# josiahls/pybullet-gym

Measured on AMD Instinct MI355X. Metric: env steps/sec (whole node) at N parallel envs, Ant + Humanoid, 1/2/4/8 MI355X, higher is better.
Workload: dtype f64

## Files before the change

### pybullet-gym_amd/csrc/pbg_robot.hip

```cpp
#include <hip/hip_runtime.h>

#include "pbg_launch.h"
#include "pbg_step.hip"
#include "pbg_team.hip"
#include "pbg_gang.hip"

#ifndef PBG_ROBOT
#error "compile with -DPBG_ROBOT=<robot struct name>"
#endif
#define PBG_CAT2(a, b) a##b
#define PBG_CAT(a, b) PBG_CAT2(a, b)
#define PBG_FN(prefix) PBG_CAT(prefix, PBG_ROBOT)

namespace pbg {
using R = pbg_models::PBG_ROBOT;
using R64 = F64<R>;
using R64L = F64L<R>;

static inline unsigned blocks(int n, int b) { return (unsigned)((n + b - 1) / b); }

static int kernel_attrs(const void* fn, Geometry* g) {
  hipFuncAttributes a{};
  const hipError_t e = hipFuncGetAttributes(&a, fn);
  g->vgprs = e == hipSuccess ? a.numRegs : -1;
  g->scratch_bytes = e == hipSuccess ? (int)a.localSizeBytes : -1;
  return (int)e;
}

template <class RR>
static int plan_team(int n_envs, int cus, Geometry* g) {
  if constexpr (Team<RR>::ok) {
    using RW = TRows<RR, 16>;
    constexpr int ES = 16;
    constexpr size_t WB = sizeof(real_t<RR>);
    const int wgs = (n_envs + ES - 1) / ES;
    const int wpc = (wgs + cus - 1) / cus;
    const size_t budget = (size_t)163840 / (size_t)(wpc > 0 ? wpc : 1);
    long words = (long)(budget / ((size_t)ES * WB)) - RW::HEAD;
    int cap = (int)(words / RW::W);
    if (cap > RW::MR) cap = RW::MR;
    if (cap < 0) cap = 0;
    size_t per_env = (size_t)RW::HEAD + (size_t)cap * RW::W;
    if (per_env < (size_t)(2 * RR::NL + 2 * RR::NJ)) per_env = 2 * RR::NL + 2 * RR::NJ;
    g->team = 4;
    g->env_words = 0;
    g->block = 64;
    g->lds_rows = cap;
    g->lds_bytes = (size_t)ES * WB * per_env;
    g->scratch_words_per_env = RW::WORDS;
    g->word_bytes = (int)WB;
    const void* fn = (const void*)team_step_kernel<RR, 16>;
    const int e = (int)hipFuncSetAttribute(fn, hipFuncAttributeMaxDynamicSharedMemorySize, (int)g->lds_bytes);
    return e ? e : kernel_attrs(fn, g);
  } else {
    (void)n_envs; (void)cus; (void)g;
    return (int)hipErrorInvalidValue;
  }
}
template <class RR>
static bool launch_team(const Buffers& B, const StepIO& io, float* scratch, const Geometry& g, hipStream_t s) {
  if constexpr (Team<RR>::ok) {
    if (g.team != 4) return false;
    hipLaunchKernelGGL((team_step_kernel<RR, 16>), dim3(blocks(4 * B.n, 64)), dim3(64), g.lds_bytes, s, B, io, scratch,
                       g.lds_rows);
    return true;
  } else {
    (void)B; (void)io; (void)scratch; (void)g; (void)s;
    return false;
  }
}

template <class RR, int T>
constexpr bool gang_ok() {
  constexpr bool f64 = sizeof(real_t<RR>) == 8;
  return (RR::kind == 0 || RR::kind >= 2) && (!RR::harder || FP<RR>::NF > 0) && (T == 16 || gang32_ok<RR>()) &&
         !(f64 && gang_big<RR>() && T != 16);
}
template <class RR, int T>
constexpr bool gang_repl() {
  return T == 16 && !RR::harder && (sizeof(real_t<RR>) == 4 || RR::NDOF < 8);
}
template <class RR, int T>
static int plan_gang_t(int n_envs, int cus, Geometry* g) {
  if constexpr (gang_ok<RR, T>()) {
    using G = Gang<RR, T>;
    constexpr long WB = (long)sizeof(real_t<RR>);
    constexpr int EPB = gang_block<RR, T>() / T;
    static_assert(4L * GangTabs<RR>::WORDS + WB * EPB * ((G::FIXED + G::MIN_CONTACT_WORDS + 3L) & ~3L) <= 163840L,
                  "gang env regions exceed the CU's LDS");
    auto region = [&](int c) {
      const int w = G::FIXED + (c * G::PERC > G::MIN_CONTACT_WORDS ? c * G::PERC : G::MIN_CONTACT_WORDS);
      return (w + G::REGION_ALIGN - 1) & ~(G::REGION_ALIGN - 1);
    };
    const int wgs = (n_envs + EPB - 1) / EPB;
    int wpc = (wgs + cus - 1) / cus;
    const long fit0 = 163840L / (4L * (long)GangTabs<RR>::WORDS + WB * EPB * (long)region(0));
    if (wpc > fit0) wpc = fit0 > 0 ? (int)fit0 : 1;
    long budget = 163840L / (long)(wpc > 0 ? wpc : 1) - 4L * (long)GangTabs<RR>::WORDS;
    if (budget < 0) budget = 0;
    long words = budget / (long)(EPB * WB) - G::FIXED;
    int cap = (int)(words / G::PERC);
    if (cap > G::MAXC) cap = G::MAXC;
    if (cap < 0) cap = 0;
    while (cap > 0 && (long)region(cap) * EPB * WB > budget) cap--;
    constexpr bool REPL = gang_repl<RR, T>();
    g->gang_dist = !REPL || RR::NDOF >= 8 || (size_t)n_envs * T > (size_t)64 * 4 * cus;
    if ((g->force_dist == 0 || g->force_dist == 1) && REPL) g->gang_dist = g->force_dist;
    g->team = T;
    g->block = gang_block<RR, T>();
    g->lds_rows = cap;
    g->env_words = region(cap);
    g->lds_bytes = 4 * (size_t)GangTabs<RR>::WORDS + (size_t)WB * (size_t)EPB * (size_t)g->env_words;
    if (g->lds_bytes > (size_t)163840) return (int)hipErrorInvalidConfiguration;
    g->scratch_words_per_env = G::GWORDS;
    g->word_bytes = (int)WB;
    const void* fn;
    if constexpr (REPL)
      fn = g->gang_dist ? (const void*)gang_step_kernel<RR, T, true> : (const void*)gang_step_kernel<RR, T, false>;
    else
      fn = (const void*)gang_step_kernel<RR, T, true>;
    const int e = (int)hipFuncSetAttribute(fn, hipFuncAttributeMaxDynamicSharedMemorySize, (int)g->lds_bytes);
    return e ? e : kernel_attrs(fn, g);
  } else {
    (void)n_envs; (void)cus; (void)g;
    return (int)hipErrorInvalidValue;
  }
}
template <class RR>
static int plan_gang(int n_envs, int cus, Geometry* g, int lanes) {
  if (lanes < 0) lanes = 16;
  if (lanes == 32) return plan_gang_t<RR, 32>(n_envs, cus, g);
  return plan_gang_t<RR, 16>(n_envs, cus, g);
}
template <class RR, int T>
static bool launch_gang_t(const Buffers& B, const StepIO& io, float* scratch, const Geometry& g, hipStream_t s) {
  if constexpr (gang_ok<RR, T>()) {
    const dim3 grid(blocks(B.n, gang_block<RR, T>() / T)), blk(gang_block<RR, T>());
    if constexpr (gang_repl<RR, T>()) {
      if (!g.gang_dist) {
        hipLaunchKernelGGL((gang_step_kernel<RR, T, false>), grid, blk, g.lds_bytes, s, B, io, scratch, g.lds_rows,
                           g.env_words);
        return true;
      }
    }
    hipLaunchKernelGGL((gang_step_kernel<RR, T, true>), grid, blk, g.lds_bytes, s, B, io, scratch, g.lds_rows, g.env_words);
    return true;
  } else {
    (void)B; (void)io; (void)scratch; (void)g; (void)s;
    return false;
  }
}
template <class RR>
static bool launch_gang(const Buffers& B, const StepIO& io, float* scratch, const Geometry& g, hipStream_t s) {
  if (g.team == 16) return launch_gang_t<RR, 16>(B, io, scratch, g, s);
  if (g.team == 32) return launch_gang_t<RR, 32>(B, io, scratch, g, s);
  return false;
}

template <class RR>
constexpr bool lane_ok() {
#ifdef PBG_DEV_GANG_ONLY
  return false;
#else
  return RR::NS <= 128;
#endif
}
template <class RR>
static int plan_lane(int n_envs, int cus, Geometry* g) {
  if constexpr (lane_ok<RR>()) {
    g->team = 1;
    g->env_words = 0;
    const int per_cu = (n_envs + cus - 1) / cus;
    int b = 16;
    while (b < per_cu && b < 64) b *= 2;
    const int wgs = (n_envs + b - 1) / b;
    const int wpc = (wgs + cus - 1) / cus;
    const size_t budget = (size_t)163840 / (size_t)(wpc > 0 ? wpc : 1);
    using RW = Rows<RR, 64>;
    constexpr size_t WB = sizeof(real_t<RR>);
    long words = (long)(budget / ((size_t)b * WB)) - RW::NC - RW::LIMW;
    int cap = (int)(words / RW::W);
    if (cap > RW::MR) cap = RW::MR;
    if (cap < 0) cap = 0;
    g->block = b;
    g->lds_rows = cap;
    g->lds_bytes = (size_t)b * WB * ((size_t)RW::LIMW + (size_t)cap * RW::W + RW::NC);
    g->scratch_words_per_env = RW::WORDS;
    g->word_bytes = (int)WB;
    const void* fn = b == 64 ? (const void*)step_kernel<RR, 64> : (b == 32 ? (const void*)step_kernel<RR, 32> : (const void*)step_kernel<RR, 16>);
    const int e = (int)hipFuncSetAttribute(fn, hipFuncAttributeMaxDynamicSharedMemorySize, (int)g->lds_bytes);
    return e ? e : kernel_attrs(fn, g);
  } else {
    (void)n_envs; (void)cus; (void)g;
    return (int)hipErrorInvalidValue;
  }
}
template <class RR>
static int launch_lane(const Buffers& B, const StepIO& io, float* scratch, const Geometry& g, hipStream_t s) {
  if constexpr (lane_ok<RR>()) {
    const dim3 grid(blocks(B.n, g.block)), blk(g.block);
    if (g.block == 64) hipLaunchKernelGGL((step_kernel<RR, 64>), grid, blk, g.lds_bytes, s, B, io, scratch, g.lds_rows);
    else if (g.block == 32) hipLaunchKernelGGL((step_kernel<RR, 32>), grid, blk, g.lds_bytes, s, B, io, scratch, g.lds_rows);
    else hipLaunchKernelGGL((step_kernel<RR, 16>), grid, blk, g.lds_bytes, s, B, io, scratch, g.lds_rows);
    return (int)hipGetLastError();
  } else {
    (void)B; (void)io; (void)scratch; (void)g; (void)s;
    return (int)hipErrorInvalidValue;
  }
}

template <class RR>
constexpr bool team64_ok() { return Team<RR>::ok; }
int PBG_FN(plan_team64_)(int n_envs, int cus, Geometry* g);
bool PBG_FN(launch_team64_)(const Buffers& B, const StepIO& io, float* scratch, const Geometry& g, hipStream_t s);
int PBG_FN(debug_stamps_t64_)(unsigned long long* host_out);
#ifdef PBG_TEAM64_TU
int PBG_FN(debug_stamps_t64_)(unsigned long long* host_out) {
#ifdef PBG_STAMPS
  if (hipMemcpyFromSymbol(host_out, HIP_SYMBOL(g_stamps), sizeof(unsigned long long) * 16) != hipSuccess) return -3;
  unsigned long long z[16] = {0};
  if (hipMemcpyToSymbol(HIP_SYMBOL(g_stamps), z, sizeof(z)) != hipSuccess) return -3;
  return 0;
#else
  (void)host_out;
  return -1;
#endif
}
#ifdef PBG_TRACE64
extern "C" int pbg_debug_trace64(double* host_out) {
  if (hipMemcpyFromSymbol(host_out, HIP_SYMBOL(g_trace64), sizeof(g_trace64)) != hipSuccess) return -3;
  return (int)(sizeof(g_trace64) / sizeof(double));
}
#endif
int PBG_FN(plan_team64_)(int n_envs, int cus, Geometry* g) {
  if constexpr (team64_ok<R64>()) return plan_team<R64>(n_envs, cus, g);
  else { (void)n_envs; (void)cus; (void)g; return (int)hipErrorInvalidValue; }
}
bool PBG_FN(launch_team64_)(const Buffers& B, const StepIO& io, float* scratch, const Geometry& g, hipStream_t s) {
  if constexpr (team64_ok<R64>()) return launch_team<R64>(B, io, scratch, g, s);
  else { (void)B; (void)io; (void)scratch; (void)g; (void)s; return false; }
}
#else

int PBG_FN(plan_)(int n_envs, int cus, int mode, Geometry* g) {
  if (Team<R>::ok && mode == 1) return plan_team<R>(n_envs, cus, g);
  if (R::kind != 1 && (mode >= 1 || !lane_ok<R>())) return plan_gang<R>(n_envs, cus, g, g->gang_lanes);
  return plan_lane<R>(n_envs, cus, g);
}

int PBG_FN(launch_step_)(const Buffers& B, const StepIO& io, float* scratch, const Geometry& g, hipStream_t s) {
  if (launch_team<R>(B, io, scratch, g, s)) return (int)hipGetLastError();
  if (launch_gang<R>(B, io, scratch, g, s)) return (int)hipGetLastError();
  return launch_lane<R>(B, io, scratch, g, s);
}

int PBG_FN(launch_reset_)(const Buffers& B, const ResetIO& io, hipStream_t s) {
  hipLaunchKernelGGL(reset_kernel<R>, dim3(blocks(B.n, 64)), dim3(64), 0, s, B, io);
  return (int)hipGetLastError();
}

int PBG_FN(launch_get_state_)(const Buffers& B, double* phys, double* aux, hipStream_t s) {
  hipLaunchKernelGGL(get_state_kernel<R>, dim3(blocks(B.n, 64)), dim3(64), 0, s, B, phys, aux);
  return (int)hipGetLastError();
}

int PBG_FN(launch_set_state_)(const Buffers& B, const double* phys, const double* aux, hipStream_t s) {
  hipLaunchKernelGGL(set_state_kernel<R>, dim3(blocks(B.n, 64)), dim3(64), 0, s, B, phys, aux);
  return (int)hipGetLastError();
}

int PBG_FN(launch_pack_)(int n, const double* in, double* out, hipStream_t s) {
  hipLaunchKernelGGL(pack_kernel<R>, dim3(blocks(n, 64)), dim3(64), 0, s, n, in, out);
  return (int)hipGetLastError();
}

int PBG_FN(plan64_)(int n_envs, int cus, int mode, Geometry* g) {
  if (team64_ok<R64>() && mode == 1) return PBG_FN(plan_team64_)(n_envs, cus, g);
  if constexpr (gang_ok<R64, 16>()) {
    if (mode != 0) {
      if (g->gang_lanes == 32 || (g->gang_lanes < 0 && gang_ok<R64, 32>())) {
        if constexpr (gang_ok<R64, 32>()) return plan_gang_t<R64, 32>(n_envs, cus, g);
        else return (int)hipErrorInvalidValue;
      }
      return plan_gang_t<R64, 16>(n_envs, cus, g);
    }
  }
  return plan_lane<R64L>(n_envs, cus, g);
}
int PBG_FN(launch_step64_)(const Buffers& B, const StepIO& io, float* scratch, const Geometry& g, hipStream_t s) {
  if (PBG_FN(launch_team64_)(B, io, scratch, g, s)) return (int)hipGetLastError();
  if (launch_gang<R64>(B, io, scratch, g, s)) return (int)hipGetLastError();
  return launch_lane<R64L>(B, io, scratch, g, s);
}
int PBG_FN(launch_reset64_)(const Buffers& B, const ResetIO& io, hipStream_t s) {
  hipLaunchKernelGGL(reset_kernel<R64>, dim3(blocks(B.n, 64)), dim3(64), 0, s, B, io);
  return (int)hipGetLastError();
}
int PBG_FN(launch_get_state64_)(const Buffers& B, double* phys, double* aux, hipStream_t s) {
  hipLaunchKernelGGL(get_state_kernel<R64>, dim3(blocks(B.n, 64)), dim3(64), 0, s, B, phys, aux);
  return (int)hipGetLastError();
}
int PBG_FN(launch_set_state64_)(const Buffers& B, const double* phys, const double* aux, hipStream_t s) {
  hipLaunchKernelGGL(set_state_kernel<R64>, dim3(blocks(B.n, 64)), dim3(64), 0, s, B, phys, aux);
  return (int)hipGetLastError();
}

int PBG_FN(debug_stamps_)(unsigned long long* host_out) {
#ifdef PBG_STAMPS
  if (hipMemcpyFromSymbol(host_out, HIP_SYMBOL(g_stamps), sizeof(unsigned long long) * 16) != hipSuccess) return -3;
  unsigned long long z[16] = {0};
  if (hipMemcpyToSymbol(HIP_SYMBOL(g_stamps), z, sizeof(z)) != hipSuccess) return -3;
  unsigned long long t64[16];
  if (PBG_FN(debug_stamps_t64_)(t64) == 0)
    for (int i = 0; i < 16; i++) host_out[i] += t64[i];
  return 0;
#else
  (void)host_out;
  return -1;
#endif
}
#endif
}
```

### pybullet-gym_amd/csrc/pbg_team.hip

```cpp

namespace pbg {

#define PBG_QUAD_SYNC                                    \
  {                                                      \
    __builtin_amdgcn_fence(__ATOMIC_RELEASE, "wavefront"); \
    __builtin_amdgcn_wave_barrier();                     \
    __builtin_amdgcn_fence(__ATOMIC_ACQUIRE, "wavefront"); \
  }

#ifdef PBG_TRACE64
#define PBG_TRACE_PH 8
__device__ double g_trace64[256][PBG_TRACE_PH][8];
#define TRACE64(ph, i, v) \
  do { if constexpr (sizeof(Sc) == 8) g_trace64[(blockIdx.x * 64 + threadIdx.x) & 255][ph][i] = (double)(v); } while (0)
#else
#define TRACE64(ph, i, v) do {} while (0)
#endif

template <int N, class S = float>
struct BTab {
  S v[N > 0 ? N : 1][4];
};
template <int N>
struct BTabI {
// ... 974 lines not shown
        fwd6(Lbb, Ldb, y6);
        Sc D2 = 0.f;
  #pragma unroll
        for (int gg = 0; gg < 6; gg++) { D2 += y6[gg] * y6[gg]; }
        Sc z[NDB];
  #pragma unroll
        for (int a = 0; a < NDB; a++) z[a] = 0.f;
        rw.put(3 * n0 + dir, -1, z, y6, D2 > Sc(1e-12) ? fast_rcp(D2) : 0.f,
               dir == 0 ? (pos_target(dist, P.k_contact, P.k_sep)) : 0.f, (Sc)R::slot_mu[sl]);
      }
      n0++;
    });
    detect_branch();
  } else {
    static_for<0, T::NS0>([&](auto sl_c) {
      constexpr int sl = decltype(sl_c)::value;
      if (!((base_bits >> sl) & 1u)) return;
      const f3 cc = O + mulc(Rb, (Sc)R::slot_point[sl][0], (Sc)R::slot_point[sl][1], (Sc)R::slot_point[sl][2]);
      const Sc rad = (Sc)R::slot_radius[sl];
      const Sc dist = cc.z - rad;
      const f3 rP = mk3<Sc>(cc.x, cc.y, cc.z - rad) - O;
      const int r0 = __builtin_popcount(base_bits & ((1u << sl) - 1u));
#pragma unroll
      for (int dir = 0; dir < 3; dir++) {
        const f3 nd = dir == 0 ? mk3<Sc>(0, 0, 1) : (dir == 1 ? mk3<Sc>(0, -1, 0) : mk3<Sc>(1, 0, 0));
        const f3 mm = cross3(rP, nd);
        Sc y6[6] = {nd.x, nd.y, nd.z, mm.x, mm.y, mm.z};
        fwd6(Lbb, Ldb, y6);
        Sc D2 = 0.f;
#pragma unroll
        for (int gg = 0; gg < 6; gg++) { D2 += y6[gg] * y6[gg]; }
        Sc z[NDB];
#pragma unroll
        for (int a = 0; a < NDB; a++) z[a] = 0.f;
        rw.put(3 * r0 + dir, -1, z, y6, D2 > Sc(1e-12) ? fast_rcp(D2) : 0.f,
               dir == 0 ? (pos_target(dist, P.k_contact, P.k_sep)) : 0.f, (Sc)R::slot_mu[sl]);
      }
    });
  }
  static_for<0, T::NSB>([&](auto sl_c) {
    constexpr int sl = decltype(sl_c)::value;
    if (!((act >> sl) & 1u)) return;
    constexpr int li = R::slot_link[T::NS0 + sl];
    const Sc dist = sdist[sl];
    const f3 rP = sP[sl] - O;
#pragma unroll
    for (int dir = 0; dir < 3; dir++) {
      const f3 nd = dir == 0 ? mk3<Sc>(0, 0, 1) : (dir == 1 ? mk3<Sc>(0, -1, 0) : mk3<Sc>(1, 0, 0));
      const f3 mm = cross3(rP, nd);
      Sc y[NDB];
      static_for<0, NDB>([&](auto a_c) {
        constexpr int a = decltype(a_c)::value;
        if constexpr (!T::in_chain(a, li)) {
          y[a] = 0.f;
        } else {
          Sc t = dot3(nd, sv[a]) + dot3(mm, sw[a]);
          static_for<0, a>([&](auto k_c) {
            constexpr int kk = decltype(k_c)::value;
            if constexpr (T::coupled(a, kk) && T::in_chain(kk, li)) t -= Lbr[a][kk] * y[kk];
          });
          y[a] = t * Ld[a];
        }
      });
      Sc y6[6] = {nd.x, nd.y, nd.z, mm.x, mm.y, mm.z};
#pragma unroll
      for (int gg = 0; gg < 6; gg++) {
#pragma unroll
        for (int b = 0; b < NDB; b++) y6[gg] -= Lgb[gg][b] * y[b];
      }
      fwd6(Lbb, Ldb, y6);
      Sc D2 = 0.f;
#pragma unroll
      for (int a = 0; a < NDB; a++) { D2 += y[a] * y[a]; }
#pragma unroll
      for (int gg = 0; gg < 6; gg++) { D2 += y6[gg] * y6[gg]; }
      rw.put(3 * ci + dir, kb, y, y6, D2 > Sc(1e-12) ? fast_rcp(D2) : 0.f,
             dir == 0 ? (pos_target(dist, P.k_contact, P.k_sep)) : 0.f, pk<T::SMU, sl>(L));
    }
    ci++;
  });
  if constexpr (OWN) lim_setup();
  if (3 * nc > rw.cap) {
    __builtin_amdgcn_fence(__ATOMIC_RELEASE, "workgroup");
    __builtin_amdgcn_fence(__ATOMIC_ACQUIRE, "workgroup");
  }
  PBG_QUAD_SYNC
  if constexpr (OWN && NLIMB > 0) {
    TRACE64(5, 0, Om[0]); TRACE64(5, 1, Orm[0]); TRACE64(5, 2, Otl[0]); TRACE64(5, 3, Oth[0]);
    TRACE64(5, 4, BY[0][0][0]); TRACE64(5, 5, BY[1][0][1]); TRACE64(5, 6, Byb[0][0][0]); TRACE64(5, 7, Om[NLIMB - 1]);
  }
  const bool all_lds = __builtin_amdgcn_ballot_w64(3 * nc > rw.cap) == 0;

  STAMP(4)
  Sc uBs[2] = {kb == 0 ? uB[0] : (kb == 1 ? uB[1] : (kb == 2 ? uB[2] : uB[3])),
                  kb == 0 ? uB[4] : (kb == 1 ? uB[5] : 0.f)};
  auto limit_sweep = [&]() {
    static_for<0, 4>([&](auto k_c) {
      constexpr int kk = decltype(k_c)::value;
      static_for<0, NLIMB>([&](auto l_c) {
        constexpr int li = decltype(l_c)::value;
        Sc part = BY[kk][li][0] * uBs[0] + BY[kk][li][1] * uBs[1];
        static_for<0, NDB>([&](auto a_c) {
          constexpr int a = decltype(a_c)::value;
          if constexpr (T::lim_nz(li, a)) part += Byb[kk][li][a] * ub[a];
        });
        const Sc yu = quad_sum(part);
        Sc dl;
        if constexpr (OWN) {
          const Sc meff = Om[li], llo = Olo[li], lhi = Ohi[li];
          const Sc nlo = clampf(llo + meff * (Otl[li] - yu), 0.f, (Sc)PBG_LIMIT_MAX_IMPULSE);
          const Sc dlo = nlo - llo;
          const Sc yu2 = yu + dlo * Orm[li];
          const Sc nhi = clampf(lhi + meff * (Oth[li] + yu2), 0.f, (Sc)PBG_LIMIT_MAX_IMPULSE);
          const Sc dhi = nhi - lhi;
          if (kb == kk) { Olo[li] = nlo; Ohi[li] = nhi; }
          dl = quad_bcast<kk>(dlo - dhi);
        } else {
          const Sc meff = Bm[kk][li], llo = Blo[kk][li], lhi = Bhi[kk][li];
          const Sc nlo = clampf(llo + meff * (Btl[kk][li] - yu), 0.f, (Sc)PBG_LIMIT_MAX_IMPULSE);
          const Sc dlo = nlo - llo;
          const Sc yu2 = yu + dlo * Brm[kk][li];
          const Sc nhi = clampf(lhi + meff * (Bth[kk][li] + yu2), 0.f, (Sc)PBG_LIMIT_MAX_IMPULSE);
          const Sc dhi = nhi - lhi;
          Blo[kk][li] = nlo;
          Bhi[kk][li] = nhi;
          dl = dlo - dhi;
        }
        uBs[0] += BY[kk][li][0] * dl;
        uBs[1] += BY[kk][li][1] * dl;
        static_for<0, NDB>([&](auto a_c) {
          constexpr int a = decltype(a_c)::value;
          if constexpr (T::lim_nz(li, a)) ub[a] += Byb[kk][li][a] * dl;
        });
      });
    });
  };
  if (all_lds) {
    for (int it = 0; it < P.iterations; it++) {
      limit_sweep();
      STAMP(11)
      contact_sweep<true>(rw, nc, kb, ub, uBs SUB_STAMP_PASS);
      STAMP(13)
    }
  } else {
    for (int it = 0; it < P.iterations; it++) {
      limit_sweep();
      STAMP(11)
      contact_sweep<false>(rw, nc, kb, ub, uBs SUB_STAMP_PASS);
      STAMP(13)
    }
  }
  {
    const Sc s0 = uBs[0], s1 = uBs[1];
    uB[0] = quad_bcast<0>(s0); uB[1] = quad_bcast<1>(s0); uB[2] = quad_bcast<2>(s0); uB[3] = quad_bcast<3>(s0);
    uB[4] = quad_bcast<0>(s1); uB[5] = quad_bcast<1>(s1);
  }
  TRACE64(6, 0, uBs[0]); TRACE64(6, 1, uBs[1]); TRACE64(6, 2, ub[0]); TRACE64(6, 3, ub[NDB - 1]);
  TRACE64(6, 4, uB[0]); TRACE64(6, 5, uB[5]); TRACE64(6, 6, nc); TRACE64(6, 7, uB[2]);

  STAMP(5)
  static_for<0, 6>([&](auto r_c) {
    constexpr int gg = 5 - decltype(r_c)::value;
    Sc t = uB[gg];
    static_for<gg + 1, 6>([&](auto h_c) { t -= Lbb[decltype(h_c)::value][gg] * nB[decltype(h_c)::value]; });
    nB[gg] = clampf(t * Ldb[gg], -(Sc)PBG_MAX_COORD_VELOCITY, (Sc)PBG_MAX_COORD_VELOCITY);
  });
  static_for<0, NDB>([&](auto r_c) {
    constexpr int a = NDB - 1 - decltype(r_c)::value;
    Sc t = ub[a];
    static_for<a + 1, NDB>([&](auto k_c) {
      constexpr int kk = decltype(k_c)::value;
      if constexpr (T::coupled(kk, a)) t -= Lbr[kk][a] * nb[kk];
    });
#pragma unroll
    for (int gg = 0; gg < 6; gg++) t -= Lgb[gg][a] * nB[gg];
    nb[a] = t * Ld[a];
  });
  static_for<0, NDB>([&](auto j_c) {
    constexpr int j = decltype(j_c)::value;
    s.qd[j] = clampf(nb[T::lg(j)], -(Sc)PBG_MAX_COORD_VELOCITY, (Sc)PBG_MAX_COORD_VELOCITY);
    s.q[j] += dt * s.qd[j];
  });
#pragma unroll
  for (int i = 0; i < 3; i++) {
    s.bv[i] = nB[i];
    s.bw[i] = nB[3 + i];
    s.bp[i] += dt * s.bv[i];
  }
  {
    const f3 wv = mk3<Sc>(s.bw[0], s.bw[1], s.bw[2]);
    Sc ang = norm3(wv);
    if (ang * dt > (Sc)PBG_ANGULAR_MOTION_THRESHOLD) ang = P.ang_max;
    Sc sh, dw;
    sincos_fast(Sc(0.5f) * ang * dt, &sh, &dw);
    f3 ax;
    if (ang < Sc(0.001)) ax = (Sc(0.5f) * dt - P.dt3c * ang * ang) * wv;
    else ax = (sh / ang) * wv;
    const Sc x = s.bq[0], y = s.bq[1], z = s.bq[2], ww = s.bq[3];
    const Sc nx = dw * x + ax.x * ww + ax.y * z - ax.z * y;
    const Sc ny = dw * y - ax.x * z + ax.y * ww + ax.z * x;
    const Sc nz = dw * z + ax.x * y - ax.y * x + ax.z * ww;
    const Sc nw = dw * ww - ax.x * x - ax.y * y - ax.z * z;
    const Sc inv = fast_rsq(nx * nx + ny * ny + nz * nz + nw * nw);
    s.bq[0] = nx * inv; s.bq[1] = ny * inv; s.bq[2] = nz * inv; s.bq[3] = nw * inv;
  }
  TRACE64(7, 0, nB[0]); TRACE64(7, 1, nB[3]); TRACE64(7, 2, nb[0]); TRACE64(7, 3, nb[NDB - 1]);
  TRACE64(7, 4, s.qd[0]); TRACE64(7, 5, s.bv[2]); TRACE64(7, 6, s.bw[0]); TRACE64(7, 7, s.bq[3]);
  STAMP(6)
  return nc;
}

template <class R, int ES>
PBG_DEV void team_gather(const TState<R>& s, const Lane& L, const TRows<R, ES>& rw, bool has_floor, PackIn<R>& in) {
  using T = Team<R>;
  using Sc = real_t<R>;
  using f3 = V3<Sc>;
  using m3 = M3<Sc>;
  constexpr int NL = R::NL, NJ = R::NJ, NDB = T::NDB, NLB = T::NLB;
  const m3 Rb = quat_to_m3(s.bq[0], s.bq[1], s.bq[2], s.bq[3]);
  TKin<R> k;
  team_fk<R>(s, L, Rb, k);
  PBG_QUAD_SYNC
#pragma unroll
  for (int i = 0; i < NLB; i++) {
    rw.stage(L.k * NLB + i) = k.c[i].x;
    rw.stage(NL + L.k * NLB + i) = k.c[i].y;
  }
#pragma unroll
  for (int j = 0; j < NDB; j++) {
    rw.stage(2 * NL + L.k * NDB + j) = s.q[j];
    rw.stage(2 * NL + NJ + L.k * NDB + j) = s.qd[j];
  }
  PBG_QUAD_SYNC
  int np = 0;
#pragma unroll
  for (int p = 0; p < R::NP; p++) {
    const int l = R::part_link[p];
    in.part_x[np] = l < 0 ? (double)s.bp[0] : (double)rw.stage(l);
    in.part_y[np] = l < 0 ? (double)s.bp[1] : (double)rw.stage(NL + l);
    np++;
  }
  if (R::floor && has_floor) { in.part_x[np] = 0.0; in.part_y[np] = 0.0; np++; }
  in.n_parts = np;
#pragma unroll
  for (int i = 0; i < 4; i++) in.quat[i] = s.bq[i];
#pragma unroll
  for (int i = 0; i < 3; i++) { in.pos[i] = s.bp[i]; in.vel[i] = s.bv[i]; in.avel[i] = s.bw[i]; }
#pragma unroll
  for (int i = 0; i < R::NO; i++) {
    in.jq[i] = rw.stage(2 * NL + R::obs_dof[i]);
    in.jqd[i] = rw.stage(2 * NL + NJ + R::obs_dof[i]);
  }
}

template <class R, int ES>
PBG_DEV void team_reset(const Buffers& B, int e, const Lane& L, TState<R>& s, const TRows<R, ES>& rw, float* obs,
                        bool& has_floor, double& pot, real_t<R>& z0) {
  using T = Team<R>;
  using Sc = real_t<R>;
#pragma unroll
  for (int i = 0; i < 3; i++) s.bp[i] = (Sc)R::base_pos[i];
#pragma unroll
  for (int i = 0; i < 4; i++) s.bq[i] = (Sc)R::base_quat[i];
#pragma unroll
  for (int i = 0; i < 3; i++) { s.bv[i] = 0.f; s.bw[i] = 0.f; }
  const uint32_t epi = B.episode[e];
  const uint32_t gid = (uint32_t)(B.env_offset + e);
  float noise[R::NR > 0 ? R::NR : 1];
#pragma unroll
  for (int blk = 0; blk < (R::NR + 3) / 4; blk++) {
    u4 ctr = {gid, epi, (uint32_t)blk, 0x5EEDu};
    const u4 rnd = philox4x32_10(ctr, (uint32_t)B.seed, (uint32_t)(B.seed >> 32));
    const uint32_t rr[4] = {rnd.x, rnd.y, rnd.z, rnd.w};
#pragma unroll
    for (int t = 0; t < 4; t++)
      if (4 * blk + t < R::NR) noise[4 * blk + t] = fmaf(0.2f, u01(rr[t]), -0.1f);
  }
  static_for<0, T::NDB>([&](auto j_c) {
    constexpr int j = decltype(j_c)::value;
    const int r = pki<T::RST, j>(L);
    Sc q = 0.f;
#pragma unroll
    for (int t = 0; t < R::NR; t++) q = r == t ? noise[t] : q;
    s.q[j] = q;
    s.qd[j] = 0.f;
  });
  PackIn<R> in;
  in.env_dt = sp_of<R>(B).env_dt;
  team_gather<R, ES>(s, L, rw, has_floor, in);
#pragma unroll
  for (int f = 0; f < R::NF; f++) in.feet_prev[f] = 0.f;
  in.feet_new = 0;
  in.potential_old = 0.0;
  in.initial_z = R::initial_z_fixed;
  PackOut po;
  if constexpr (R::kind == 3) mujoco3d_pack<R>(in, nullptr, obs, po);
  else walker_pack<R>(in, nullptr, obs, po);
  pot = po.potential;
  z0 = (Sc)po.initial_z;
  has_floor = true;
  if (L.k == 0) B.episode[e] = epi + 1;
}

template <class R, int ES>
__global__ __launch_bounds__(64) void team_step_kernel(Buffers B, StepIO io, float* __restrict__ scratch, int lds_rows) {
  using T = Team<R>;
  using Sc = real_t<R>;
  using LW = lds_t<Sc>;
  constexpr int NDB = T::NDB, SB = PBG_BASE_WORDS;
  extern __shared__ float lds_dyn[];
  const int tid = xcd_block() * blockDim.x + threadIdx.x;
  const int e = tid >> 2;
  if (e >= B.n) return;
  const Lane L = make_lane(tid & 3);
  const int kb = L.k;
  STAMP_DECL
  TState<R> s;
#pragma unroll
  for (int i = 0; i < 3; i++) s.bp[i] = st_of<R>(B)[(size_t)i * B.n + e];
#pragma unroll
  for (int i = 0; i < 4; i++) s.bq[i] = st_of<R>(B)[(size_t)(3 + i) * B.n + e];
#pragma unroll
  for (int i = 0; i < 3; i++) s.bv[i] = st_of<R>(B)[(size_t)(7 + i) * B.n + e];
#pragma unroll
  for (int i = 0; i < 3; i++) s.bw[i] = st_of<R>(B)[(size_t)(10 + i) * B.n + e];
#pragma unroll
  for (int j = 0; j < NDB; j++) {
    s.q[j] = st_of<R>(B)[(size_t)(SB + kb * NDB + j) * B.n + e];
    s.qd[j] = st_of<R>(B)[(size_t)(SB + R::NJ + kb * NDB + j) * B.n + e];
  }
  constexpr bool LATE = sizeof(Sc) == 8;
  int el = 0;
  uint32_t flags = 0;
  double pot_old = 0.0;
  Sc z0_old = 0.f;
  auto book = [&]() {
    el = B.elapsed[e] + 1;
    flags = B.flags[e];
    pot_old = B.pot[e];
    z0_old = z0_of<R>(B)[e];
  };
  if constexpr (!LATE) book();
  float act[R::NA];
#pragma unroll
  for (int i = 0; i < R::NA; i++) act[i] = io.act[(size_t)e * R::NA + i];
  Sc tau[NDB];
  static_for<0, NDB>([&](auto j_c) {
    constexpr int j = decltype(j_c)::value;
    const int ai = pki<T::ACTI, j>(L);
    float a = 0.f;
#pragma unroll
    for (int i = 0; i < R::NA; i++) a = ai == i ? act[i] : a;
    tau[j] = ai < 0 ? 0.f : (Sc)((double)pk<T::GAIN, j>(L) * (double)fminf(fmaxf(a, -1.f), 1.f));
  });
  TRows<R, ES> rw;
  rw.lds = (LW*)lds_dyn + (threadIdx.x >> 2);
  rw.rows = (LW*)lds_dyn + TRows<R, ES>::HEAD * ES;
  rw.lane = threadIdx.x;
  rw.gbl = (Sc*)scratch + e;
  rw.n = B.n;
  rw.cap = lds_rows;
  uint32_t slot_bits = 0, base_bits = 0;
  int nc = 0;
  STAMP(7)
  uint32_t csig = 0;
  for (int sub = 0; sub < sp_of<R>(B).substeps; sub++) {
    nc = team_substep<R, ES>(s, L, tau, slot_bits, base_bits, rw, sp_of<R>(B) SUB_STAMP_PASS);
    if (io.csig) {
      if (kb == 0)
        for (int sl = 0; sl < T::NS0; sl++)
          if ((base_bits >> sl) & 1u) csig += pbg_contact_hash((uint32_t)sub, (uint32_t)sl);
      for (int sl = 0; sl < T::NSB; sl++)
        if ((slot_bits >> sl) & 1u) csig += pbg_contact_hash((uint32_t)sub, (uint32_t)(T::NS0 + kb * T::NSB + sl));
    }
  }
  if (io.ncontact && kb == 0) io.ncontact[e] = nc;
  if (io.csig) {
    uint32_t sig = csig;
    sig += (uint32_t)qperm_i<0xB1>((int)sig);
    sig += (uint32_t)qperm_i<0x4E>((int)sig);
    if (kb == 0) io.csig[e] = sig;
  }
  if constexpr (LATE) {
    book();
    const float* ap = io.act;
    asm volatile("" : "+s"(ap));
#pragma unroll
    for (int i = 0; i < R::NA; i++) act[i] = ap[(size_t)e * R::NA + i];
  }
  uint32_t fb = 0;
  static_for<0, T::NSB>([&](auto sl_c) {
    constexpr int sl = decltype(sl_c)::value;
    constexpr int li = R::slot_link[T::NS0 + sl];
    const int f = pki<T::FOOT, li>(L);
    if (f >= 0 && ((slot_bits >> sl) & 1u)) fb |= 1u << f;
  });
  const uint32_t fnew = (uint32_t)quad_sum_i((int)fb);
  float obs[R::OBS];
  PackOut po;
  {
    PackIn<R> in;
    in.env_dt = sp_of<R>(B).env_dt;
    team_gather<R, ES>(s, L, rw, flags & 1u, in);
#pragma unroll
    for (int f = 0; f < R::NF; f++) in.feet_prev[f] = ((flags >> (8 + f)) & 1u) ? 1.f : 0.f;
    in.feet_new = fnew;
    in.potential_old = pot_old;
    in.initial_z = z0_old;
    if constexpr (R::kind == 3) mujoco3d_pack<R>(in, act, obs, po);
    else walker_pack<R, false, 4>(in, act, obs, po, kb);
    flags = (flags & 0xFFu) | (po.feet_out << 8);
  }
  STAMP(8)
  int eo = e;
  if constexpr (sizeof(Sc) == 8) asm volatile("" : "+v"(eo));
  const bool term = po.done;
  const bool trunc = el >= R::max_episode_steps;
  if (kb == 0) {
    io.rew[eo] = (float)po.reward;
    if (io.rew64) io.rew64[eo] = po.reward;
    if (io.rew_terms) {
#pragma unroll
      for (int i = 0; i < 5; i++) io.rew_terms[(size_t)eo * 5 + i] = po.terms[i];
    }
    io.done[eo] = term || trunc;
    if (io.trunc) io.trunc[eo] = trunc && !term;
  }
  if (io.autoreset && (term || trunc)) {
    if (io.term_obs) lanes_store_row<R, 4>(obs, io.term_obs, eo, kb);
    bool has_floor = flags & 1u;
    double pot;
    Sc z0;
    team_reset<R, ES>(B, eo, L, s, rw, obs, has_floor, pot, z0);
    if (kb == 0) {
      B.pot[eo] = pot;
      z0_of<R>(B)[eo] = z0;
      B.elapsed[eo] = 0;
      B.flags[eo] = has_floor ? 1u : 0u;
    }
  } else if (kb == 0) {
    B.pot[eo] = po.potential;
    B.elapsed[eo] = el;
    B.flags[eo] = flags;
  }
  {
    const Sc bw[PBG_BASE_WORDS] = {s.bp[0], s.bp[1], s.bp[2], s.bq[0], s.bq[1], s.bq[2], s.bq[3],
                                      s.bv[0], s.bv[1], s.bv[2], s.bw[0], s.bw[1], s.bw[2]};
    static_for<0, (PBG_BASE_WORDS + 3) / 4>([&](auto m_c) {
      constexpr int m = decltype(m_c)::value;
      const Sc v = lanes_pick<4, m, PBG_BASE_WORDS>(bw, kb);
      if (4 * m + kb < PBG_BASE_WORDS) st_of<R>(B)[(size_t)(4 * m + kb) * B.n + eo] = v;
    });
    lanes_store_row<R, 4>(obs, io.obs, eo, kb);
  }
#pragma unroll
  for (int j = 0; j < NDB; j++) {
    st_of<R>(B)[(size_t)(SB + kb * NDB + j) * B.n + eo] = s.q[j];
    st_of<R>(B)[(size_t)(SB + R::NJ + kb * NDB + j) * B.n + eo] = s.qd[j];
  }
  STAMP(9)
  STAMP_FLUSH
}

}
```

### pybullet-gym_amd/csrc/pbg_types.h

```cpp
#pragma once
#include <stdint.h>

#include <type_traits>

namespace pbg {
template <class S>
struct SimPT {
  S dt;
  S gravity;
  S k_sep;
  S k_contact;
  S k_limit;
  S ang_max;
  S dt3c;
  int substeps;
  int iterations;
  int flag_timeout;
  double env_dt;
};
using SimP = SimPT<float>;

template <class S = float>
inline SimPT<S> resolve_sim_params(double timestep, int frame_skip, int iterations, double gravity, double contact_erp,
                                   double limit_erp, double angular_motion_threshold) {
  SimPT<S> p;
  p.dt = (S)timestep;
  const S inv_dt = (S)(1.0 / timestep);
  p.gravity = (S)gravity;
  p.k_sep = -inv_dt;
  p.k_contact = -(S)contact_erp * inv_dt;
  p.k_limit = -(S)limit_erp * inv_dt;
  p.ang_max = (S)angular_motion_threshold / p.dt;
  p.dt3c = p.dt * p.dt * p.dt * (sizeof(S) == 4 ? (S)0.020833333333f : (S)0.020833333333);
  p.substeps = frame_skip;
  p.iterations = iterations;
  p.flag_timeout = (600 + frame_skip - 1) / frame_skip;
  p.env_dt = timestep * frame_skip;
  return p;
}

template <class R, class = void>
struct RealOf {
  using type = float;
};
template <class R>
struct RealOf<R, std::void_t<typename R::real>> {
  using type = typename R::real;
};
template <class R>
using real_t = typename RealOf<R>::type;
template <class R0>
struct F64 : R0 {
  using real = double;
};
template <class R0>
struct F64L : F64<R0> {
#ifdef PBG_DEV_LANE_OWN_TRIG
  static constexpr bool lib_trig = false;
#else
  static constexpr bool lib_trig = true;
#endif
};
template <class R, class = void>
struct LibTrig {
  static constexpr bool value = false;
};
template <class R>
struct LibTrig<R, std::void_t<decltype(R::lib_trig)>> {
  static constexpr bool value = R::lib_trig;
};
template <class R>
inline constexpr bool lib_trig_v = LibTrig<R>::value;

struct Buffers {
  int n;
  void* st;
  double* pot;
  void* z0;
  int* elapsed;
  uint32_t* flags;
  uint32_t* episode;
  double* tgt;
  int32_t* ftm;
  double* hkd;
  int32_t* hki;
  uint64_t seed;
  int env_offset;
  SimP sp;
  SimPT<double> sp64;
};

struct StepIO {
  const float* act;
  float* obs;
  float* rew;
  double* rew64;
  uint8_t* done;
  uint8_t* trunc;
  float* term_obs;
  int32_t* ncontact;
  int autoreset;
  double* rew_terms;
  uint32_t* csig;
};

struct ResetIO {
  const uint8_t* mask;
  const float* init_q;
  float* obs;
};

}
```

Baseline: 217.9 million.

## Restructure team-step epilogue stores: early state writeback, 16-byte obs rows, lane-split scalars

Writes the physics state back right after the substep loop, or after the late action load, so those stores overlap with observation packing. Stores observation rows as 16-byte vectors per lane when the output pointer is aligned. Per-env scalar outputs (done/trunc, reward/elapsed/flags) are spread across the four team lanes instead of all coming from lane 0. Reset envs rewrite state after an explicit vmcnt wait, which adds a redundant store and a stall on that path.

```diff
diff --git a/pybullet-gym_amd/csrc/pbg_robot.hip b/pybullet-gym_amd/csrc/pbg_robot.hip
--- a/pybullet-gym_amd/csrc/pbg_robot.hip
+++ b/pybullet-gym_amd/csrc/pbg_robot.hip
@@ -61,7 +61,10 @@
 static bool launch_team(const Buffers& B, const StepIO& io, float* scratch, const Geometry& g, hipStream_t s) {
   if constexpr (Team<RR>::ok) {
     if (g.team != 4) return false;
-    hipLaunchKernelGGL((team_step_kernel<RR, 16>), dim3(blocks(4 * B.n, 64)), dim3(64), g.lds_bytes, s, B, io, scratch,
+    auto al16 = [](const void* p) { return p != nullptr && ((uintptr_t)p & 15u) == 0; };
+    StepIO w = io;
+    w.wide = (al16(io.obs) ? PBG_WIDE_OBS : 0u) | (al16(io.term_obs) ? PBG_WIDE_TERM_OBS : 0u);
+    hipLaunchKernelGGL((team_step_kernel<RR, 16>), dim3(blocks(4 * B.n, 64)), dim3(64), g.lds_bytes, s, B, w, scratch,
                        g.lds_rows);
     return true;
   } else {
diff --git a/pybullet-gym_amd/csrc/pbg_team.hip b/pybullet-gym_amd/csrc/pbg_team.hip
--- a/pybullet-gym_amd/csrc/pbg_team.hip
+++ b/pybullet-gym_amd/csrc/pbg_team.hip
@@ -1300,6 +1300,56 @@
   if (L.k == 0) B.episode[e] = epi + 1;
 }
 
+typedef float qf4 __attribute__((ext_vector_type(4)));
+typedef uint32_t __attribute__((may_alias)) qu32;
+
+template <int W, int I>
+PBG_DEV float quad_pick4(const float (&v)[W], int t) {
+  const float a = v[I], b = v[I + 4 < W ? I + 4 : I], c = v[I + 8 < W ? I + 8 : I], d = v[I + 12 < W ? I + 12 : I];
+  float r = a;
+  r = t == 1 ? b : r;
+  r = t == 2 ? c : r;
+  r = t == 3 ? d : r;
+  return r;
+}
+template <int W>
+PBG_DEV void quad_store_row16(const float (&v)[W], float* __restrict__ out, int e, int t) {
+  static_assert(W % 4 == 0, "a row of whole 16-byte pieces");
+  static_for<0, (W + 15) / 16>([&](auto m_c) {
+    constexpr int m = decltype(m_c)::value;
+    const float x0 = quad_pick4<W, 16 * m + 0>(v, t), x1 = quad_pick4<W, 16 * m + 1>(v, t);
+    const float x2 = quad_pick4<W, 16 * m + 2>(v, t), x3 = quad_pick4<W, 16 * m + 3>(v, t);
+    if (16 * m + 4 * t < W) *(qf4*)(out + (size_t)e * W + 16 * m + 4 * t) = qf4{x0, x1, x2, x3};
+  });
+}
+template <class R>
+PBG_DEV void quad_store_row(const float (&obs)[R::OBS], float* __restrict__ out, int e, int t, bool wide) {
+  if constexpr (R::OBS % 4 == 0) {
+    if (wide) {
+      quad_store_row16<R::OBS>(obs, out, e, t);
+      return;
+    }
+  }
+  lanes_store_row<R, 4>(obs, out, e, t);
+}
+template <class R>
+PBG_DEV void quad_store_state(const Buffers& B, const TState<R>& s, int e, int kb) {
+  using Sc = real_t<R>;
+  constexpr int NDB = Team<R>::NDB, SB = PBG_BASE_WORDS;
+  const Sc bw[PBG_BASE_WORDS] = {s.bp[0], s.bp[1], s.bp[2], s.bq[0], s.bq[1], s.bq[2], s.bq[3],
+                                 s.bv[0], s.bv[1], s.bv[2], s.bw[0], s.bw[1], s.bw[2]};
+  static_for<0, (PBG_BASE_WORDS + 3) / 4>([&](auto m_c) {
+    constexpr int m = decltype(m_c)::value;
+    const Sc v = lanes_pick<4, m, PBG_BASE_WORDS>(bw, kb);
+    if (4 * m + kb < PBG_BASE_WORDS) st_of<R>(B)[(size_t)(4 * m + kb) * B.n + e] = v;
+  });
+#pragma unroll
+  for (int j = 0; j < NDB; j++) {
+    st_of<R>(B)[(size_t)(SB + kb * NDB + j) * B.n + e] = s.q[j];
+    st_of<R>(B)[(size_t)(SB + R::NJ + kb * NDB + j) * B.n + e] = s.qd[j];
+  }
+}
+
 template <class R, int ES>
 __global__ __launch_bounds__(64) void team_step_kernel(Buffers B, StepIO io, float* __restrict__ scratch, int lds_rows) {
   using T = Team<R>;
@@ -1372,6 +1422,12 @@
         if ((slot_bits >> sl) & 1u) csig += pbg_contact_hash((uint32_t)sub, (uint32_t)(T::NS0 + kb * T::NSB + sl));
     }
   }
+  auto early_state_store = [&]() {
+    int ee = e;
+    if constexpr (sizeof(Sc) == 8) asm volatile("" : "+v"(ee));
+    quad_store_state<R>(B, s, ee, kb);
+  };
+  if constexpr (!LATE) early_state_store();
   if (io.ncontact && kb == 0) io.ncontact[e] = nc;
   if (io.csig) {
     uint32_t sig = csig;
@@ -1383,9 +1439,11 @@
     book();
     const float* ap = io.act;
     asm volatile("" : "+s"(ap));
-#pragma unroll
-    for (int i = 0; i < R::NA; i++) act[i] = ap[(size_t)e * R::NA + i];
-  }
+    const __attribute__((address_space(1))) float* gp = (const __attribute__((address_space(1))) float*)ap;
+#pragma unroll
+    for (int i = 0; i < R::NA; i++) act[i] = gp[(size_t)e * R::NA + i];
+  }
+  if constexpr (LATE) early_state_store();
   uint32_t fb = 0;
   static_for<0, T::NSB>([&](auto sl_c) {
     constexpr int sl = decltype(sl_c)::value;
@@ -1415,47 +1473,40 @@
   const bool term = po.done;
   const bool trunc = el >= R::max_episode_steps;
   if (kb == 0) {
-    io.rew[eo] = (float)po.reward;
     if (io.rew64) io.rew64[eo] = po.reward;
     if (io.rew_terms) {
 #pragma unroll
       for (int i = 0; i < 5; i++) io.rew_terms[(size_t)eo * 5 + i] = po.terms[i];
     }
-    io.done[eo] = term || trunc;
-    if (io.trunc) io.trunc[eo] = trunc && !term;
-  }
+  }
+  int el_out = el;
+  uint32_t flags_out = flags;
+  double pot_out = po.potential;
   if (io.autoreset && (term || trunc)) {
-    if (io.term_obs) lanes_store_row<R, 4>(obs, io.term_obs, eo, kb);
+    if (io.term_obs) quad_store_row<R>(obs, io.term_obs, eo, kb, io.wide & PBG_WIDE_TERM_OBS);
     bool has_floor = flags & 1u;
     double pot;
     Sc z0;
     team_reset<R, ES>(B, eo, L, s, rw, obs, has_floor, pot, z0);
-    if (kb == 0) {
-      B.pot[eo] = pot;
-      z0_of<R>(B)[eo] = z0;
-      B.elapsed[eo] = 0;
-      B.flags[eo] = has_floor ? 1u : 0u;
-    }
-  } else if (kb == 0) {
-    B.pot[eo] = po.potential;
-    B.elapsed[eo] = el;
-    B.flags[eo] = flags;
+    if (kb == 0) z0_of<R>(B)[eo] = z0;
+    el_out = 0;
+    flags_out = has_floor ? 1u : 0u;
+    pot_out = pot;
+    asm volatile("s_waitcnt vmcnt(0)" ::: "memory");
+    quad_store_state<R>(B, s, eo, kb);
   }
   {
-    const Sc bw[PBG_BASE_WORDS] = {s.bp[0], s.bp[1], s.bp[2], s.bq[0], s.bq[1], s.bq[2], s.bq[3],
-                                      s.bv[0], s.bv[1], s.bv[2], s.bw[0], s.bw[1], s.bw[2]};
-    static_for<0, (PBG_BASE_WORDS + 3) / 4>([&](auto m_c) {
-      constexpr int m = decltype(m_c)::value;
-      const Sc v = lanes_pick<4, m, PBG_BASE_WORDS>(bw, kb);
-      if (4 * m + kb < PBG_BASE_WORDS) st_of<R>(B)[(size_t)(4 * m + kb) * B.n + eo] = v;
-    });
-    lanes_store_row<R, 4>(obs, io.obs, eo, kb);
-  }
-#pragma unroll
-  for (int j = 0; j < NDB; j++) {
-    st_of<R>(B)[(size_t)(SB + kb * NDB + j) * B.n + eo] = s.q[j];
-    st_of<R>(B)[(size_t)(SB + R::NJ + kb * NDB + j) * B.n + eo] = s.qd[j];
-  }
+    uint8_t* p = kb == 0 ? io.done : io.trunc;
+    const uint8_t v = kb == 0 ? (term || trunc) : (trunc && !term);
+    if (kb == 0 || (kb == 1 && io.trunc)) p[eo] = v;
+  }
+  {
+    qu32* p = kb == 0 ? (qu32*)io.rew : (kb == 1 ? (qu32*)B.elapsed : (qu32*)B.flags);
+    const uint32_t v = kb == 0 ? __float_as_uint((float)po.reward) : (kb == 1 ? (uint32_t)el_out : flags_out);
+    if (kb < 3) p[eo] = v;
+  }
+  if (kb == 0) B.pot[eo] = pot_out;
+  quad_store_row<R>(obs, io.obs, eo, kb, io.wide & PBG_WIDE_OBS);
   STAMP(9)
   STAMP_FLUSH
 }
diff --git a/pybullet-gym_amd/csrc/pbg_types.h b/pybullet-gym_amd/csrc/pbg_types.h
--- a/pybullet-gym_amd/csrc/pbg_types.h
+++ b/pybullet-gym_amd/csrc/pbg_types.h
@@ -102,7 +102,9 @@
   int autoreset;
   double* rew_terms;
   uint32_t* csig;
+  uint32_t wide = 0;
 };
+enum : uint32_t { PBG_WIDE_OBS = 1u, PBG_WIDE_TERM_OBS = 2u };
 
 struct ResetIO {
   const uint8_t* mask;
```

Result: no change. 217.6 million (-0.1%).
